# sen-ye/dmvae

Measured on AMD Instinct MI355X. Metric: images/sec DMVAE train step @256x256, higher is better.
Workload: dtype bf16

## Files before the change

### dmvae_amd/_lib.py

```python
from __future__ import annotations

import ctypes
import os
from ctypes import POINTER, Structure, c_char_p, c_float, c_int, c_int32, c_longlong, c_size_t, c_uint, c_ulonglong, c_void_p

_HERE = os.path.dirname(os.path.abspath(__file__))
LIB_PATH = os.environ.get("DMVAE_LIB") or os.path.join(_HERE, "libdmvae_hip.so")


class ConvDesc(Structure):
    _fields_ = [("n", c_int32), ("h", c_int32), ("w", c_int32), ("cin", c_int32), ("cout", c_int32),
                ("ks", c_int32), ("upsample", c_int32), ("act", c_int32), ("out_f32", c_int32), ("stride", c_int32), ("transposed", c_int32),
                ("w_layout", c_int32)]


class PackEntry(Structure):
    _fields_ = [("src", c_void_p), ("dst", c_void_p), ("dst2", c_void_p),
                ("cout", c_int32), ("cin", c_int32), ("T", c_int32), ("rows_pad", c_int32), ("cols_pad", c_int32), ("mode", c_int32), ("subpixel", c_int32),
                ("reserved", c_int32), ("start", c_ulonglong), ("count", c_ulonglong)]


class WtEntry(Structure):
    _fields_ = [("src", c_void_p), ("dst", c_void_p), ("N", c_int32), ("K", c_int32), ("start", c_uint), ("tiles_x", c_uint)]


class OdeTerms(Structure):
    _fields_ = [("k", c_void_p * 7), ("c", c_float * 7), ("nk", c_int32), ("k_bf16", c_int32)]


ABI_VERSION = 9

SIGNATURES = {
    "dmvae_last_error": (c_char_p, []),
    "dmvae_abi_version": (c_int, []),
    "dmvae_rms_modulate_fwd_f32": (c_int, [c_void_p] * 6 + [c_size_t, c_int, c_int, c_int, c_float, c_void_p]),
    "dmvae_rms_modulate_bwd_f32": (c_int, [c_void_p] * 8 + [c_size_t, c_int, c_int, c_int, c_void_p]),
    "dmvae_layernorm_bwd_full_f32": (c_int, [c_void_p] * 5 + [c_size_t, c_int, c_float, c_void_p]),
    "dmvae_bcast_rows_f32": (c_int, [c_int] + [c_void_p] * 4 + [c_size_t, c_int, c_int, c_int, c_void_p]),
    "dmvae_colsum_groups_f32": (c_int, [c_void_p, c_void_p, c_int, c_int, c_int, c_int, c_void_p]),
    "dmvae_swiglu_fwd_f32": (c_int, [c_void_p, c_void_p, c_size_t, c_int, c_void_p]),
    "dmvae_swiglu_bwd_f32": (c_int, [c_void_p, c_void_p, c_void_p, c_size_t, c_int, c_void_p]),
    "dmvae_qknorm_rope_fwd_f32": (c_int, [c_void_p] * 9 + [c_int] * 5 + [c_float, c_void_p]),
    "dmvae_qknorm_rope_bwd_f32": (c_int, [c_void_p] * 12 + [c_int] * 5 + [c_void_p]),
    "dmvae_reparam_kl_workspace": (c_size_t, [c_size_t, c_int]),
    "dmvae_reparam_kl_fwd": (c_int, [c_void_p] * 5 + [c_size_t, c_size_t, c_int, c_int, c_void_p]),
    "dmvae_reparam_kl_bwd": (c_int, [c_void_p] * 4 + [c_float, c_void_p, c_size_t, c_int, c_int, c_void_p]),
    "dmvae_conv2d_nhwc_fwd": (c_int, [c_void_p, c_void_p, c_void_p, c_void_p, c_void_p, POINTER(ConvDesc), c_void_p]),
    "dmvae_conv2d_nhwc_fwd_gnstats_workspace": (c_size_t, [POINTER(ConvDesc), c_int]),
    "dmvae_conv2d_nhwc_fwd_gnstats": (c_int, [c_void_p] * 7 + [c_size_t, c_int, c_float, POINTER(ConvDesc), c_void_p]),
    "dmvae_conv2d_nhwc_wgrad_workspace": (c_size_t, [POINTER(ConvDesc)]),
    "dmvae_gemm_nt_batched": (c_int, [c_void_p] * 5 + [c_int] * 4 + [c_longlong] * 3 + [c_int, c_int, c_void_p]),
    "dmvae_gemm_tn_batched_workspace": (c_size_t, [c_int, c_int, c_int, c_int]),
    "dmvae_gemm_tn_batched": (c_int, [c_void_p] * 4 + [c_size_t] + [c_int] * 4 + [c_longlong] * 3 + [c_float, c_int, c_void_p]),
    "dmvae_set_dynamic": (c_int, [c_int]),
    "dmvae_linear_rows_supported": (c_int, [c_int, c_int, c_int]),
    "dmvae_linear_rows_bf16": (c_int, [c_void_p] * 4 + [c_int] * 10 + [c_void_p]),
    "dmvae_linear_rows_wgrad": (c_int, [c_void_p] * 4 + [c_int] * 6 + [c_void_p]),
    "dmvae_linear_bf16": (c_int, [c_void_p] * 4 + [c_int] * 10 + [c_void_p]),
    "dmvae_linear_bf16_swiglu_pre": (c_int, [c_void_p] * 5 + [c_int] * 9 + [c_void_p]),
    "dmvae_linear_bf16_sk_supported": (c_int, [c_int] * 5),
    "dmvae_linear_bf16_sk_workspace": (c_size_t, [c_int] * 5),
    "dmvae_linear_bf16_sk": (c_int, [c_void_p] * 5 + [c_size_t] + [c_int] * 11 + [c_void_p]),
    "dmvae_linear_bf16_batched_supported": (c_int, [c_int] * 4),
    "dmvae_linear_bf16_batched": (c_int, [c_void_p] * 3 + [c_int] * 7 + [c_longlong] * 3 + [c_int, c_void_p]),
    "dmvae_linear_bf16_plan": (c_int, [c_int, c_int, c_int, POINTER(c_int), POINTER(c_int)]),
    "dmvae_linear_weight_t_kmajor": (c_int, [c_void_p, c_void_p, c_int, c_int, c_void_p]),
    "dmvae_pack_entry_bytes": (c_size_t, []),
    "dmvae_pack_weights_batched": (c_int, [c_void_p, c_int, c_ulonglong, c_int, c_void_p]),
    "dmvae_softmax_rows_fwd": (c_int, [c_void_p, c_void_p, c_int, c_int, c_float, c_void_p]),
    "dmvae_softmax_rows_bwd": (c_int, [c_void_p, c_void_p, c_void_p, c_int, c_int, c_float, c_void_p]),
    "dmvae_transpose_bf16": (c_int, [c_void_p, c_void_p, c_int, c_int, c_int, c_void_p]),
    "dmvae_pack_conv_weight": (c_int, [c_void_p, c_void_p] + [c_int] * 6 + [c_void_p]),
    "dmvae_pack_conv_weight_v2": (c_int, [c_void_p, c_void_p, c_void_p] + [c_int] * 6 + [c_void_p]),
    "dmvae_conv_halo_applies": (c_int, [POINTER(ConvDesc)]),
    "dmvae_conv_kmajor_applies": (c_int, [POINTER(ConvDesc)]),
    "dmvae_subpixel_weight": (c_int, [c_void_p, c_void_p, c_int, c_int, c_void_p]),
    "dmvae_subpixel_weight_fold": (c_int, [c_void_p, c_void_p, c_int, c_int, c_int, c_void_p]),
    "dmvae_colsum_bf16": (c_int, [c_void_p, c_void_p, c_void_p, c_size_t, c_size_t, c_int, c_int, c_void_p]),
    "dmvae_conv_out_wgrad_workspace": (c_size_t, [c_int, c_int, c_int, c_int, c_int]),
    "dmvae_conv_out_wgrad": (c_int, [c_void_p, c_void_p, c_void_p, c_void_p, c_size_t, c_int, c_int, c_int, c_int, c_int, c_int, c_void_p]),
    "dmvae_sumpool2x2_nhwc": (c_int, [c_void_p, c_void_p, c_int, c_int, c_int, c_int, c_void_p]),
    "dmvae_maxpool2x2_nhwc": (c_int, [c_void_p, c_void_p, c_int, c_int, c_int, c_int, c_void_p]),
    "dmvae_maxpool2x2_relu_bwd_nhwc": (c_int, [c_void_p, c_void_p, c_void_p, c_void_p, c_int, c_int, c_int, c_int, c_void_p]),
    "dmvae_relu_bwd": (c_int, [c_void_p, c_void_p, c_void_p, c_size_t, c_void_p]),
    "dmvae_leaky_relu_bwd": (c_int, [c_void_p, c_void_p, c_void_p, c_size_t, c_float, c_void_p]),
    "dmvae_sde_euler_step": (c_int, [c_void_p, c_void_p, c_int, c_void_p, c_void_p, c_void_p, c_size_t] + [c_float] * 6 + [c_void_p]),
    "dmvae_image_to_u8": (c_int, [c_void_p, c_void_p, c_size_t, c_int, c_int, c_int, c_void_p]),
# ... 159 lines not shown
```

### dmvae_amd/csrc/conv_pp.hip

```cpp
#include "common.h"
#include "dmvae_hip.h"
#include <cstdlib>
#include <atomic>
#include <mutex>
#include <type_traits>
#include <unordered_map>


namespace dmvae_conv_pp {

struct Args {
  const bf16* x;
  const bf16* w;
  const float* bias;
  const bf16* res;
  void* y;
  int N, Hi, Wi, Cin, Ho, Wo, Cout;
  int ks, act, M, ctiles, total;
  int so, pd, sd;
  int Ml;
  unsigned wsRow, wsTap, wsChunk;
  float* gnpart;
  unsigned* sched;
  unsigned long long* dbg;
};

__device__ __forceinline__ int hswz(int row) { return (row >> 1) & 2; }

__device__ __forceinline__ void divmod_small(int m, int d, float inv_d, bool, int& q, int& r) {
  q = (int)((float)m * inv_d);
  r = m - q * d;
  if (r < 0) { q--; r += d; }
  if (r >= d) { q++; r -= d; }
}

template <int TM, int TP, int WM, int WP, int NBUF, bool UPS, bool OUT_F32, bool KO, bool GEN = false, bool SUB = false, bool DYN = false, bool STATS = false,
          bool HALO = false>
__global__ __launch_bounds__(512) void conv_pp_kernel(Args a) {
#if __HIP_DEVICE_COMPILE__
  constexpr int BM = TM / WM / 32, BP = TP / WP / 32;
  constexpr int TILE_A = TM * 64, TILE_B = TP * 64, SLOT = TILE_A + TILE_B;
  constexpr int NPA = TM >= 128 ? TM / 128 : 1, NPB = TP / 128;
  static_assert(TM >= 128 || HALO, "the 64-row tile exists in the halo form only");
  constexpr int NP = NPA + NPB;
  constexpr int PF = NBUF - 1;
  static_assert(WM * WP == 8 && BM * BP == 8, "8 waves x 8 accumulators");
  static_assert(!HALO || (!UPS && !GEN && !SUB && KO && NBUF == 4), "HALO: plain 3x3, chunk-outer K order");
  constexpr int NPH = NPB + 1;
  constexpr int HALO_B = (TP + 16) * 64;
  constexpr int GROUP = 2 * TILE_A + HALO_B;
  constexpr int EPI_OFF = HALO ? GROUP : 2 * SLOT;
  constexpr int EPI_BYTES = 8 * 32 * (((BM >= 4 ? BM / 2 : BM) * 32) * 4 + 16);
  constexpr int DUMP_OFF = GROUP + (GROUP > EPI_BYTES ? GROUP : EPI_BYTES);
  constexpr bool DIRECT = HALO && !OUT_F32;
  constexpr int BM16 = BM * 2, BP16 = BP * 2;
  extern __shared__ __attribute__((aligned(16))) char smem[];

  const int tid = threadIdx.x, lane = tid & 63;
  const int wave = __builtin_amdgcn_readfirstlane(tid >> 6);
  const int grp = wave >> 2;
  const int wm = wave / WP, wp = wave % WP;
  static_assert(!SUB || (!UPS && !GEN && KO), "SUB: its own instantiation, chunk-outer K order");
  const int T = SUB ? 4 : a.ks * a.ks;
  const int TW = SUB ? 16 : T;
  const int nchunk = a.Cin >> 5;
  const int nK = T * nchunk;

  const unsigned wbytes = (unsigned)a.Cout * TW * a.Cin * 2u;
  const unsigned xbytes = (unsigned)a.N * a.Hi * a.Wi * a.Cin * 2u;
  const int SR = GEN ? ((UPS || a.ks == 1) ? 0 : (a.sd == 2 ? 1 : a.pd)) : 1;
  const int sds = GEN && a.sd == 2 ? 1 : 0;
  const unsigned shift = GEN ? ((!UPS && a.ks != 1) ? (unsigned)(SR * a.Wi + SR) * a.Cin * 2u : 0u)
                             : ((!UPS && (SUB || a.ks == 3)) ? (unsigned)(a.Wi + 1) * a.Cin * 2u : 0u);
  const __amdgpu_buffer_rsrc_t rA = dmvae_buffer_rsrc(a.w, wbytes);
  const __amdgpu_buffer_rsrc_t rB =
      dmvae_buffer_rsrc(reinterpret_cast<const char*>(a.x) - shift, xbytes + shift);

  const int dvw = SUB ? a.Wi : a.Wo;
  const int hw = SUB ? a.Hi * a.Wi : a.Ho * a.Wo;
  const float inv_hw = 1.0f / (float)hw, inv_wo = 1.0f / (float)dvw;
  const bool small_m = a.M < (1 << 24);
  int m0 = 0, n0 = 0;
  int par = 0;
  unsigned voffA[NPA];
  unsigned ctrB[NPB], maskB[NPB], selB[NPB];
  unsigned rowo[UPS ? NPB : 1][3], colo[UPS ? NPB : 1][3];
  unsigned ctrH[HALO ? NPH : 1], mskH[HALO ? NPH : 1];
// ... 1 lines not shown
  int it = 0, it_tap = 0, it_ch = 0;
  unsigned soffB_tap = 0;
  auto setup = [&](unsigned work) {
    int lane_s = lane;
    if constexpr (DIRECT) asm volatile("" : "+v"(lane_s));
    const unsigned wid = xcd_remap(work, a.total);
    if constexpr (SUB) {
      const unsigned q = wid / a.ctiles;
      n0 = (int)(wid - q * a.ctiles) * TM;
      par = __builtin_amdgcn_readfirstlane((int)(q & 3u));
      m0 = (int)(q >> 2) * TP;
    } else {
      m0 = (int)(wid / a.ctiles) * TP;
      n0 = (int)(wid % a.ctiles) * TM;
    }
    it = it_tap = it_ch = 0;
    it_ky = 0;
#pragma unroll
    for (int p = 0; p < NPA; p++) {
      const int row = (wave * NPA + p) * 16 + (lane_s >> 2);
      int co = n0 + row;
      if constexpr (DIRECT) {
        constexpr int CW_ = TM / WM;
        const int wmr = row / CW_, rr = row % CW_;
        co = n0 + wmr * CW_ + BM16 * (rr & 15) + (rr >> 4);
      }
      const int c = (lane_s & 3) ^ swz64(row);
      voffA[p] = (co < a.Cout && row < TM) ? (unsigned)co * a.wsRow + c * 16u : SENT;
    }
    if constexpr (HALO) {
#pragma unroll
      for (int q = 0; q < NPH; q++) {
        const int i = (q < NPB ? (wave * NPB + q) * 16 : TP) + (lane_s >> 2);
        const int own = min(max(i - 1, 0), TP - 1);
        const int m = m0 + own;
        const int c = (lane_s & 3) ^ hswz(i);
        unsigned mask = 0;
        if (m < a.M && i < TP + 2 && (q < NPB || wave == 0)) {
          int n, r, y, x;
          divmod_small(m, hw, inv_hw, small_m, n, r);
          divmod_small(r, dvw, inv_wo, small_m, y, x);
          mask = (y > 0 ? 1u : 0u) | 2u | (y < a.Ho - 1 ? 4u : 0u);
          if ((i == 0 && x == 0) || (i == TP + 1 && x == a.Wo - 1)) mask = 0;
        }
        ctrH[q] = (unsigned)(m0 + i) * a.Cin * 2u + c * 16u;
        mskH[q] = mask;
      }
    } else {
#pragma unroll
    for (int p = 0; p < NPB; p++) {
    const int row = (wave * NPB + p) * 16 + (lane_s >> 2);
    const int m = m0 + row;
    const int c = (lane_s & 3) ^ swz64(row);
    unsigned mask = 0;
    ctrB[p] = 0;
    if (m < a.M) {
      int n, r, y, x;
      divmod_small(m, hw, inv_hw, small_m, n, r);
      divmod_small(r, dvw, inv_wo, small_m, y, x);
      int by = y, bx = x;
      if constexpr (SUB) {
        by = y - 1 + (par >> 1); bx = x - 1 + (par & 1);
        const unsigned rm = (by >= 0 ? 0x3u : 0u) | (by + 1 < a.Hi ? 0xCu : 0u);
        const unsigned cm = (bx >= 0 ? 0x5u : 0u) | (bx + 1 < a.Wi ? 0xAu : 0u);
        mask = rm & cm;
      } else if (UPS || !GEN) {
        if (a.ks == 3) {
          const unsigned rm = (y > 0 ? 0x007u : 0u) | 0x038u | (y < a.Ho - 1 ? 0x1C0u : 0u);
          const unsigned cm = (x > 0 ? 0x049u : 0u) | 0x092u | (x < a.Wo - 1 ? 0x124u : 0u);
          mask = rm & cm;
        } else {
          mask = 1;
        }
      } else if (a.ks == 1) {
        mask = 1;
      } else {
// ... 69 lines not shown
        const unsigned co = kx == 0 ? colo[UPS ? p : 0][0] : (kx == 1 ? colo[UPS ? p : 0][1] : colo[UPS ? p : 0][2]);
        v = ro + co;
      }
      selB[p] = ((maskB[p] >> it_tap) & 1u) ? v : SENT;
    }
  };
  auto issue = [&](int slot) {
    const bool live = it < nK;
    if (live && (KO || it_ch == 0)) new_tap();
    unsigned soA = (unsigned)it_tap * a.wsTap + (unsigned)it_ch * a.wsChunk;
    if constexpr (SUB)
      soA = (unsigned)((((par >> 1) + (it_tap & 2)) << 2) + (par & 1) + ((it_tap & 1) << 1)) * a.wsTap + (unsigned)it_ch * a.wsChunk;
    unsigned soB = soffB_tap + (unsigned)it_ch * 64u;
    constexpr bool live_b = true;
    if constexpr (GEN) {
      soA = (unsigned)__builtin_amdgcn_readfirstlane((int)soA);
      soB = (unsigned)__builtin_amdgcn_readfirstlane((int)soB);
    }
#pragma unroll
    for (int p = 0; p < NPA; p++)
      __builtin_amdgcn_raw_ptr_buffer_load_lds(rA, LPTR(smem + slot + (wave * NPA + p) * 1024), 16, live ? voffA[p] : SENT, soA, 0, 0);
#pragma unroll
    for (int p = 0; p < NPB; p++)
      __builtin_amdgcn_raw_ptr_buffer_load_lds(rB, LPTR(smem + slot + TILE_A + (wave * NPB + p) * 1024), 16, (live && live_b) ? selB[p] : SENT, soB, 0, 0);
    it++;
    if (KO) {
      if (++it_tap == T) { it_tap = 0; it_ch++; }
    } else {
      if (++it_ch == nchunk) { it_ch = 0; it_tap++; }
    }
  };

  auto issue_h = [&](auto KXc) __attribute__((always_inline)) {
    constexpr int KX = decltype(KXc)::value;
    const bool live = it < nK;
    const unsigned soA = (unsigned)(it_ky * 3 + KX) * a.wsTap + (unsigned)it_ch * a.wsChunk;
    const int isl = it;
    const int da = ((isl >> 1) & 1) * GROUP + (isl & 1) * TILE_A;
#pragma unroll
    for (int p = 0; p < NPA; p++)
      __builtin_amdgcn_raw_ptr_buffer_load_lds(rA, LPTR(smem + ((wave * NPA + p) * 16 < TM ? da + (wave * NPA + p) * 1024 : DUMP_OFF)), 16, live ? voffA[p] : SENT, soA, 0, 0);
    if constexpr (KX == 0) {
      const unsigned soH = (unsigned)(it_ky * a.Wi) * a.Cin * 2u + (unsigned)it_ch * 64u;
      const int dh = ((it_ch + it_ky) & 1) * GROUP + 2 * TILE_A;
#pragma unroll
      for (int q = 0; q < NPH; q++) {
        const unsigned v = (live && ((mskH[HALO ? q : 0] >> it_ky) & 1u)) ? ctrH[HALO ? q : 0] : SENT;
        const int dst = q < NPB ? dh + (wave * NPB + q) * 1024 : (wave == 0 ? dh + TP * 64 : DUMP_OFF);
        __builtin_amdgcn_raw_ptr_buffer_load_lds(rB, LPTR(smem + dst), 16, v, soH, 0, 0);
      }
    }
    it++;
    if constexpr (KX == 2) {
      if (++it_ky == 3) { it_ky = 0; it_ch++; }
    }
  };
  using K0_ = std::integral_constant<int, 0>; using K1_ = std::integral_constant<int, 1>; using K2_ = std::integral_constant<int, 2>;

  auto stamp = [&](unsigned work, int k) {
    if (a.dbg && tid == 0) a.dbg[(size_t)work * 8 + k] = __builtin_amdgcn_s_memtime();
  };
  auto claim = [&]() {
    if (tid == 0) {
      const unsigned x = blockIdx.x & 7u, first = gridDim.x >> 3;
      unsigned flat = 0xFFFFFFFFu;
      for (unsigned k = 0; k < 8u; k++) {
        const unsigned xx = (x + k) & 7u;
        const unsigned cnt = ((unsigned)a.total >> 3) + (xx < ((unsigned)a.total & 7u) ? 1u : 0u);
        const unsigned j = first + atomicAdd(a.sched + xx, 1u);
        if (j < cnt) { flat = j * 8u + xx; break; }
      }
      __hip_atomic_store(a.sched + 16 + blockIdx.x, flat, __ATOMIC_RELEASE, __HIP_MEMORY_SCOPE_WORKGROUP);
    }
  };
  stamp(blockIdx.x, 0);
  setup(blockIdx.x);
  stamp(blockIdx.x, 1);
  if constexpr (HALO) {
    issue_h(K0_{}); issue_h(K1_{}); issue_h(K2_{});
  } else {
#pragma unroll
    for (int u = 0; u < PF; u++) issue(u * SLOT);
  }
  for (unsigned work = blockIdx.x; work < (unsigned)a.total;) {
  const int m0c = m0, n0c = n0;
  const int parc = par;
  if constexpr (DYN) claim();
  int boffk[HALO ? 3 : 1][HALO ? BP16 : 1];
  if constexpr (HALO) {
    int lane_h = lane;
    asm volatile("" : "+v"(lane_h));
#pragma unroll
    for (int j = 0; j < BP16; j++) {
      const int prow = wp * (TP / WP) + j * 16 + (lane_h & 15);
      int q, x;
      divmod_small(m0c + prow, dvw, inv_wo, small_m, q, x);
      const int zoff = (TP + 2) * 64 + ((lane_h >> 4) << 4);
#pragma unroll
      for (int k = 0; k < 3; k++) {
        const int h = prow + k;
        const int off = h * 64 + (((lane_h >> 4) ^ hswz(h)) << 4);
        boffk[HALO ? k : 0][HALO ? j : 0] = (k == 0 && x == 0) || (k == 2 && x == a.Wo - 1) ? zoff : off;
      }
    }
  }
#pragma unroll
  for (int i = 0; i < BM16; i++)
#pragma unroll
    for (int j = 0; j < BP16; j++)
#pragma unroll
      for (int r = 0; r < 4; r++) acc[i][j][r] = 0.f;
  wait_vmcnt<HALO ? 2 * NPA : (PF - 1) * NP>();
  __builtin_amdgcn_s_barrier();
  stamp(work, 2);
  if (grp == 1) __builtin_amdgcn_s_setprio(1);
  if (grp == 1) __builtin_amdgcn_s_barrier();

  bf16x8 af[BM16], bfr[BP16];
  int slot_rd = 0, slot_wr = PF * SLOT;
  unsigned next_dyn = 0;
  if constexpr (HALO) {
    int ka = 0, sh = 2 * TILE_A;
    auto ktile = [&](auto KXc) __attribute__((always_inline)) {
      constexpr int KX = decltype(KXc)::value;
      const char* sa = smem + ((ka >> 1) & 1) * GROUP + (ka & 1) * TILE_A;
      const char* sb = smem + sh;
#pragma unroll
      for (int j = 0; j < BP16; j++) bfr[j] = *reinterpret_cast<const bf16x8*>(sb + boffk[HALO ? KX : 0][HALO ? j : 0]);
#pragma unroll
      for (int i = 0; i < BM16; i++) af[i] = *reinterpret_cast<const bf16x8*>(sa + aoff[i]);
      issue_h(KXc);
      ka++;
      if constexpr (KX == 2) sh = sh == 2 * TILE_A ? GROUP + 2 * TILE_A : 2 * TILE_A;
      wait_vmcnt<KX == 2 ? 2 * NPA : 2 * NPA + NPH>();
      __builtin_amdgcn_s_waitcnt(0xC07F);
      asm volatile("" ::: "memory");
      __builtin_amdgcn_sched_barrier(0);
      __builtin_amdgcn_s_barrier();
      __builtin_amdgcn_sched_barrier(0);
#pragma unroll
      for (int i = 0; i < BM16; i++)
#pragma unroll
        for (int j = 0; j < BP16; j++) {
          if constexpr (DIRECT) asm volatile("v_mfma_f32_16x16x32_bf16 %0, %1, %2, %0" : "+a"(acc[i][j]) : "v"(bfr[j]), "v"(af[i]));
          else asm volatile("v_mfma_f32_16x16x32_bf16 %0, %1, %2, %0" : "+a"(acc[i][j]) : "v"(af[i]), "v"(bfr[j]));
        }
      __builtin_amdgcn_sched_barrier(0);
      __builtin_amdgcn_s_barrier();
      __builtin_amdgcn_sched_barrier(0);
    };
#pragma unroll 1
    for (int t = 0; t < nK; t += 3) { ktile(K0_{}); ktile(K1_{}); ktile(K2_{}); }
  } else {
#pragma unroll 1
  for (int t = 0; t < nK; t++) {
    const char* sb = smem + slot_rd;
#pragma unroll
    for (int j = 0; j < BP16; j++) bfr[j] = *reinterpret_cast<const bf16x8*>(sb + boff[j]);
#pragma unroll
    for (int i = 0; i < BM16; i++) af[i] = *reinterpret_cast<const bf16x8*>(sb + aoff[i]);
    issue(slot_wr);
    slot_rd = slot_rd + SLOT == NBUF * SLOT ? 0 : slot_rd + SLOT;
    slot_wr = slot_wr + SLOT == NBUF * SLOT ? 0 : slot_wr + SLOT;
    wait_vmcnt<(PF - 1) * NP>();
    __builtin_amdgcn_s_waitcnt(0xC07F);
    asm volatile("" ::: "memory");
    __builtin_amdgcn_sched_barrier(0);
    __builtin_amdgcn_s_barrier();
    __builtin_amdgcn_sched_barrier(0);
#pragma unroll
    for (int i = 0; i < BM16; i++)
#pragma unroll
      for (int j = 0; j < BP16; j++)
        asm volatile("v_mfma_f32_16x16x32_bf16 %0, %1, %2, %0" : "+a"(acc[i][j]) : "v"(af[i]), "v"(bfr[j]));
    __builtin_amdgcn_sched_barrier(0);
    __builtin_amdgcn_s_barrier();
    __builtin_amdgcn_sched_barrier(0);
  }
  }
  stamp(work, 3);
  if (grp == 0) __builtin_amdgcn_s_barrier();
  if constexpr (DYN) next_dyn = __hip_atomic_load(a.sched + 16 + blockIdx.x, __ATOMIC_ACQUIRE, __HIP_MEMORY_SCOPE_WORKGROUP);
  wait_vmcnt<0>();
  asm volatile("s_nop 15\n\ts_nop 15" ::: "memory");

// ... 369 lines not shown
  const unsigned long long key = ((unsigned long long)(unsigned)dev << 56) ^ (unsigned long long)reinterpret_cast<uintptr_t>(st);
  auto it = slot.find(key);
  if (it == slot.end()) {
    int& n = used[dev];
    if (n >= SCHED_SLOTS) return nullptr;
    it = slot.emplace(key, n++).first;
  }
  return b->second + (size_t)it->second * SCHED_WORDS;
}

static std::atomic<int> g_dynamic{-1};
static bool dynamic_on() {
  const int v = g_dynamic.load(std::memory_order_relaxed);
  if (v >= 0) return v != 0;
  static const bool env = [] { const char* e = getenv("DMVAE_PP_DYNAMIC"); return e ? atoi(e) != 0 : false; }();
  return env;
}

template <int TM, int TP, int WM, int WP, int NBUF, bool UPS, bool F32, bool KO, bool GEN = false, bool SUB = false, bool DYN = false, bool STATS = false,
          bool HALO = false>
int launch(Args a, hipStream_t st) {
  a.ctiles = (a.Cout + TM - 1) / TM;
  a.total = ((a.M + TP - 1) / TP) * a.ctiles * (SUB ? 4 : 1);
  constexpr int persist = 256;
  const unsigned grid = (persist > 0 && a.total > persist) ? (unsigned)persist : (unsigned)a.total;
  if constexpr (!DYN && !UPS && KO && !F32) {
    if (dynamic_on() && grid == 256u && (unsigned)a.total > grid) {
      a.sched = sched_for(st);
      if (a.sched) return launch<TM, TP, WM, WP, NBUF, UPS, F32, KO, GEN, SUB, true, STATS, HALO>(a, st);
    }
  }
  constexpr int cwh = (TM / WM / 32 >= 4) ? TM / WM / 2 : TM / WM;
  constexpr int ring = NBUF * (TM + TP) * 64, epi = 2 * (TM + TP) * 64 + 8 * 32 * (cwh * 4 + 16);
  constexpr int group = 2 * TM * 64 + (TP + 16) * 64, epi_h = 8 * 32 * (cwh * 4 + 16);
  constexpr int lds = HALO ? group + (group > epi_h ? group : epi_h) + 1024 : (ring > epi ? ring : epi);
  DMVAE_LDS_OPTIN(lds, conv_pp_kernel<TM, TP, WM, WP, NBUF, UPS, F32, KO, GEN, SUB, DYN, STATS, HALO>);
  hipLaunchKernelGGL((conv_pp_kernel<TM, TP, WM, WP, NBUF, UPS, F32, KO, GEN, SUB, DYN, STATS, HALO>), dim3(grid), dim3(512), lds, st, a);
  DMVAE_CHECK_LAUNCH();
  return 0;
}

static constexpr int halo_mode() { return 3; }
static constexpr bool korder_on() { return true; }
static bool halo_for(int ks, int cout, bool plain, bool ups, bool f32) {
  const int h = halo_mode();
  return plain && !ups && !f32 && ks == 3 && h != 0 && korder_on() && (cout > 128 || (h & 2));
}

template <bool UPS, bool F32>
int pick(const Args& a, hipStream_t st, bool gen) {
  if constexpr (!UPS) {
    if (gen) {
      if (a.Cout <= 128) return launch<128, 512, 2, 4, 4, false, F32, true, true>(a, st);
      return launch<256, 256, 2, 4, 4, false, F32, true, true>(a, st);
    }
  }
  if constexpr (UPS) {
    if (a.Cout <= 128) return launch<128, 512, 2, 4, 4, UPS, F32, false>(a, st);
    return launch<256, 256, 2, 4, 4, UPS, F32, false>(a, st);
  } else {
    if constexpr (!F32) {
      if (halo_for(a.ks, a.Cout, !gen, UPS, F32)) {
        if (a.Cout > 128) return a.gnpart ? launch<256, 256, 2, 4, 4, false, false, true, false, false, false, true, true>(a, st)
                                          : launch<256, 256, 2, 4, 4, false, false, true, false, false, false, false, true>(a, st);
        if (a.Cout <= 64 && !a.gnpart)
          return launch<64, 1024, 1, 8, 4, false, false, true, false, false, false, false, true>(a, st);
        return a.gnpart ? launch<128, 512, 2, 4, 4, false, false, true, false, false, false, true, true>(a, st)
                        : launch<128, 512, 2, 4, 4, false, false, true, false, false, false, false, true>(a, st);
      }
      if (a.gnpart) {
        if (a.Cout <= 128) return launch<128, 512, 2, 4, 4, false, false, true, false, false, false, true>(a, st);
        return launch<256, 256, 2, 4, 4, false, false, true, false, false, false, true>(a, st);
      }
    }
    if (a.Cout <= 128) return launch<128, 512, 2, 4, 4, UPS, F32, true>(a, st);
    return launch<256, 256, 2, 4, 4, UPS, F32, true>(a, st);
  }
}

}

static unsigned long long* g_dbg = nullptr;
extern "C" void dmvae_debug_timing(void* buf) { g_dbg = (unsigned long long*)buf; }

__global__ __launch_bounds__(64) void occupy_kernel(unsigned long long ticks) {
  extern __shared__ char occ[];
  occ[threadIdx.x] = 0;
  const unsigned long long t0 = wall_clock64();
  while (wall_clock64() - t0 < ticks) __builtin_amdgcn_s_sleep(32);
}
extern "C" int dmvae_set_dynamic(int on) {
  dmvae_conv_pp::g_dynamic.store(on < 0 ? -1 : (on != 0), std::memory_order_relaxed);
  return dmvae_conv_pp::dynamic_on() ? 1 : 0;
}

extern "C" int dmvae_debug_occupy(int blocks, int lds_bytes, int microseconds, hipStream_t stream) {
  DMVAE_LDS_OPTIN(160 * 1024, occupy_kernel);
  hipLaunchKernelGGL(occupy_kernel, dim3(blocks), dim3(64), lds_bytes, stream, (unsigned long long)microseconds * 100ull);
  DMVAE_CHECK_LAUNCH();
  return 0;
}

int dmvae_conv_geometry(const dmvae_conv_desc* d, int* ho, int* wo, int* so, int* pd, int* sd, int* fl);

extern "C" int dmvae_conv_halo_applies(const dmvae_conv_desc* d) {
  using namespace dmvae_conv_pp;
  if (!d) return 0;
  int ho, wo, so, pd, sd, fl;
  if (dmvae_conv_geometry(d, &ho, &wo, &so, &pd, &sd, &fl) != 0) return 0;
  const bool plain = !(d->upsample == 2 || d->stride == 2 || d->ks == 4 || d->transposed);
  const long long M = (long long)d->n * ho * wo;
  const long long xbytes = (long long)d->n * d->h * d->w * d->cin * 2;
  const long long wbytes = (long long)d->cout * d->ks * d->ks * d->cin * 2;
  constexpr long long min_m = 16384;
  if (d->cin % 32 != 0 || d->cout < 64 || d->cout % 8 != 0 || M < min_m || xbytes + (1ll << 22) >= (1ll << 31) || wbytes >= (1ll << 31)) return 0;
  if (M >= (1ll << 24) || M * d->cout * (d->out_f32 ? 4 : 2) >= (1ll << 31)) return 0;
  return halo_for(d->ks, d->cout, plain, fl != 0, d->out_f32 != 0) ? 1 : 0;
}

extern "C" int dmvae_conv_kmajor_applies(const dmvae_conv_desc* d) {
  using namespace dmvae_conv_pp;
  if (!d) return 0;
  int ho, wo, so, pd, sd, fl;
  if (dmvae_conv_geometry(d, &ho, &wo, &so, &pd, &sd, &fl) != 0) return 0;
  const bool plain = !(d->upsample == 2 || d->stride == 2 || d->ks == 4 || d->transposed);
  const long long M = (long long)d->n * ho * wo;
  const long long xbytes = (long long)d->n * d->h * d->w * d->cin * 2;
  const long long wbytes = (long long)d->cout * d->ks * d->ks * d->cin * 2;
  constexpr long long min_m = 16384;
  if (d->cin % 32 != 0 || d->cout < 64 || d->cout % 8 != 0 || M < min_m || xbytes + (1ll << 22) >= (1ll << 31) || wbytes >= (1ll << 31)) return 0;
  if (M >= (1ll << 24) || M * d->cout * (d->out_f32 ? 4 : 2) >= (1ll << 31)) return 0;
  return 1;
}

int dmvae_conv_pp_try(const void* x, const void* w, const void* bias, const void* residual, void* y, const dmvae_conv_desc* d,
                      hipStream_t stream, float* gnpart, int gn_groups, int* gn_tp) {
  if (gn_tp) *gn_tp = 0;
  using namespace dmvae_conv_pp;
  int ho, wo, so, pd, sd, fl;
  if (dmvae_conv_geometry(d, &ho, &wo, &so, &pd, &sd, &fl) != 0) return 1;
  const bool plain = !(d->upsample == 2 || d->stride == 2 || d->ks == 4 || d->transposed);
  const bool sub = d->transposed && d->ks == 4 && d->stride == 2;
  const int ups = fl ? 1 : 0;
  const long long M = (long long)d->n * ho * wo;
  const long long xbytes = (long long)d->n * d->h * d->w * d->cin * 2;
  const long long wbytes = (long long)d->cout * d->ks * d->ks * d->cin * 2;
  constexpr long long min_m = 16384;
  if (d->cin % 32 != 0 || d->cout < 64 || d->cout % 8 != 0 || M < min_m || xbytes + (1ll << 22) >= (1ll << 31) || wbytes >= (1ll << 31)) return 1;
  if (M >= (1ll << 24)) return 1;
  if (M * d->cout * (d->out_f32 ? 4 : 2) >= (1ll << 31)) return 1;
  if (d->w_layout != 0 && d->w_layout != 1) {
    dmvae_set_error("conv2d_nhwc_fwd: w_layout %d (0 = tap-major, 1 = K-tile-major where dmvae_conv_kmajor_applies(d) is 1)", d->w_layout);
    return -1;
  }
  Args a;
  a.wsRow = d->w_layout ? 64u : (unsigned)(d->ks * d->ks * d->cin) * 2u;
  a.wsTap = d->w_layout ? (unsigned)d->cout * 64u : (unsigned)d->cin * 2u;
  a.wsChunk = d->w_layout ? (unsigned)(d->ks * d->ks) * (unsigned)d->cout * 64u : 64u;
  a.x = (const bf16*)x; a.w = (const bf16*)w; a.bias = (const float*)bias; a.res = (const bf16*)residual; a.y = y;
  a.N = d->n; a.Hi = d->h; a.Wi = d->w; a.Cin = d->cin; a.Cout = d->cout;
  a.Ho = ho; a.Wo = wo; a.so = so; a.pd = pd; a.sd = sd;
  a.ks = d->ks; a.act = d->act; a.M = (int)M; a.ctiles = 0; a.dbg = g_dbg;
  a.Ml = d->n * d->h * d->w;
  a.gnpart = nullptr;
  if (gnpart && gn_tp && !d->out_f32 && (plain || sub) && !ups && gn_groups > 0 && d->cout % gn_groups == 0 && (d->cout / gn_groups) % 4 == 0) {
    const int tp = d->cout <= 128 ? 512 : 256;
    const long long per_image = sub ? (long long)d->h * d->w : (long long)ho * wo;
    if (per_image % tp == 0) { a.gnpart = gnpart; *gn_tp = tp; }
  }
  a.sched = nullptr;
  const bool f32 = d->out_f32 != 0;
  if (sub) {
    a.M = a.Ml;
    if (a.gnpart) {
      if (a.Cout <= 128) return launch<128, 512, 2, 4, 4, false, false, true, false, true, false, true>(a, stream);
      return launch<256, 256, 2, 4, 4, false, false, true, false, true, false, true>(a, stream);
    }
    if (a.Cout <= 128) return f32 ? launch<128, 512, 2, 4, 4, false, true, true, false, true>(a, stream) : launch<128, 512, 2, 4, 4, false, false, true, false, true>(a, stream);
    return f32 ? launch<256, 256, 2, 4, 4, false, true, true, false, true>(a, stream) : launch<256, 256, 2, 4, 4, false, false, true, false, true>(a, stream);
  }
  if (ups) return f32 ? pick<true, true>(a, stream, false) : pick<true, false>(a, stream, false);
  return f32 ? pick<false, true>(a, stream, !plain) : pick<false, false>(a, stream, !plain);
}
```

### dmvae_amd/ops.py

```python
from __future__ import annotations

import ctypes
import os
from typing import Optional, Sequence, Tuple

import torch

from . import _lib, parity
from ._lib import ConvDesc, check

bf16 = torch.bfloat16
f32 = torch.float32

ACT_NONE, ACT_SILU, ACT_RELU, ACT_RELU_GATE, ACT_LEAKY, ACT_GELU = 0, 1, 2, 3, 4, 5
ACT_SWIGLU = 6


def _stream() -> int:
    return torch.cuda.current_stream().cuda_stream


def _req(t: torch.Tensor, dtype, name: str) -> torch.Tensor:
    if not t.is_cuda:
        raise _lib.DmvaeHipError(f"{name}: expected a GPU tensor; dmvae_amd has no CPU path")
    if t.dtype != dtype:
        raise TypeError(f"{name}: expected {dtype}, got {t.dtype}")
    if not t.is_contiguous():
        raise ValueError(f"{name}: tensor must be contiguous")
    return t


def _ptr(t: Optional[torch.Tensor]):
    return None if t is None else t.data_ptr()


_WS = {}

KERNEL_TIMING = None
_PP_HALO = 3


def workspace(nbytes: int, device, slot: str = "main") -> torch.Tensor:
    key = (device.index if device.index is not None else torch.cuda.current_device(), _stream(), slot)
    ws = _WS.get(key)
    if ws is None or ws.numel() < nbytes:
        ws = torch.empty(max(int(nbytes), 1 << 20), dtype=torch.uint8, device=device)
        _WS[key] = ws
    return ws


def pack_conv_weight(w: torch.Tensor, for_dgrad: bool = False, rows_pad: int = 0, cols_pad: int = 0, kmajor: bool = False) -> torch.Tensor:
    if parity.on():
        return parity.pack_conv_weight(w, for_dgrad, rows_pad, cols_pad)
    w = _req(w, f32, "weight")
    if w.dim() == 2:
        cout, cin, ks = w.shape[0], w.shape[1], 1
    else:
        cout, cin, ks = w.shape[0], w.shape[1], w.shape[2]
    rows, cols = (cin, cout) if for_dgrad else (cout, cin)
    rows_pad, cols_pad = max(rows_pad, rows), max(cols_pad, cols)
    out = torch.empty(rows_pad, ks * ks, cols_pad, dtype=bf16, device=w.device)
    out2 = torch.empty(cols_pad // 32, ks * ks, rows_pad, 32, dtype=bf16, device=w.device) if (kmajor and cols_pad % 32 == 0) else None
    check(_lib.lib().dmvae_pack_conv_weight_v2(w.data_ptr(), out.data_ptr(), _ptr(out2), cout, cin, ks, rows_pad, cols_pad, int(for_dgrad), _stream()),
          "pack_conv_weight")
    if out2 is not None:
        out._dmvae_kmajor = out2
    return out


def _weight_operand(w_packed: torch.Tensor, d) -> int:
    wk = getattr(w_packed, "_dmvae_kmajor", None)
    if wk is not None and _lib.lib().dmvae_conv_kmajor_applies(ctypes.byref(d)):
# ... 14 lines not shown
def subpixel_weight_fold(dwd: torch.Tensor, dw_out: Optional[torch.Tensor] = None, accumulate: bool = False) -> torch.Tensor:
    dwd = _req(dwd, f32, "dwd")
    cin, cout = dwd.shape[0], dwd.shape[1]
    dw = dw_out if dw_out is not None else torch.empty(cout, cin, 3, 3, dtype=f32, device=dwd.device)
    assert dw.is_contiguous() and dw.numel() == cout * cin * 9
    check(_lib.lib().dmvae_subpixel_weight_fold(dwd.data_ptr(), dw.data_ptr(), cout, cin, int(accumulate), _stream()), "subpixel_weight_fold")
    return dw


def colsum(x: torch.Tensor, out: Optional[torch.Tensor] = None, accumulate: bool = False) -> torch.Tensor:
    c = x.shape[-1]
    if x.dtype == f32 and parity.on():
        s = parity.colsum(x.reshape(-1, c))
        if out is None:
            return s
        return out.add_(s) if accumulate else out.copy_(s)
    x = _req(x, bf16, "x")
    out = out if out is not None else torch.empty(c, dtype=f32, device=x.device)
    ws = workspace(512 * c * 4, x.device, slot="colsum")
    check(_lib.lib().dmvae_colsum_bf16(x.data_ptr(), out.data_ptr(), ws.data_ptr(), ws.numel(), x.numel() // c, c, int(accumulate), _stream()), "colsum_bf16")
    return out


def conv_out_size(h: int, w: int, ks: int, upsample: int = 0, stride: int = 1, transposed: bool = False):
    if ks == 4:
        return ((h - 1) * stride + 2, (w - 1) * stride + 2) if transposed else ((h - 2) // stride + 1, (w - 2) // stride + 1)
    if upsample or transposed:
        return 2 * h, 2 * w
    return (h // 2, w // 2) if stride == 2 else (h, w)


def _conv_label(n, ho, wo, cin, cout, ks, upsample, out_f32, stride, transposed, stats):
    sub = bool(transposed) and ks == 4 and stride == 2
    if cin % 32 == 0 and cout >= 64 and cout % 8 == 0 and n * ho * wo >= 16384:
        ups1 = int(upsample) == 1
        gen = (int(upsample) == 2 or stride == 2 or ks == 4 or bool(transposed)) and not sub
        t = lambda f: "true" if f else "false"
        dyn = os.environ.get("DMVAE_PP_DYNAMIC", "0") not in ("", "0") and not ups1 and not out_f32 and (n * ho * wo // (512 if cout <= 128 else 256)) * ((cout + 255) // 256 if cout > 128 else 1) > 256
        halo = ks == 3 and not gen and not sub and not ups1 and not out_f32
        label = "conv_pp_kernel<%s, %s, %s, %s, %s, %s, %s, %s, %s>" % (("64, 1024, 1, 8, 4" if (halo and cout <= 64 and not stats) else ("128, 512" if cout <= 128 else "256, 256") + ", 2, 4, 4"), t(ups1), t(out_f32),
                                                                       "false" if ups1 else "true", t(gen), t(sub), t(dyn), t(stats), t(halo))
    else:
        label = "conv_fwd_kernel"
    return label, 2.0 * n * ho * wo * cout * cin * (4 if sub else ks * ks)


def conv2d_nhwc(x: torch.Tensor, w_packed: torch.Tensor, bias: Optional[torch.Tensor] = None,
                residual: Optional[torch.Tensor] = None, ks: int = 3, upsample=False, act: int = ACT_NONE,
                out_f32: bool = False, stride: int = 1, transposed: bool = False, flop_channels: Optional[Tuple[int, int]] = None) -> torch.Tensor:
    if x.dtype == f32 and parity.on():
        y = conv2d_nhwc(parity.split_channels(x, parity.A_SIDE), w_packed, bias, None, ks, upsample, ACT_NONE, True, stride, transposed)
        return parity.epilogue(y, residual, act)
    x = _req(x, bf16, "x")
    w_packed = _req(w_packed, bf16, "w_packed")
    n, h, w_, cin = x.shape
    cout = w_packed.shape[0]
    assert w_packed.shape[1] == ks * ks and w_packed.shape[2] == cin, (w_packed.shape, ks, cin)
    ho, wo = conv_out_size(h, w_, ks, int(upsample), stride, transposed)
    y = torch.empty(n, ho, wo, cout, dtype=f32 if out_f32 else bf16, device=x.device)
    if bias is not None:
        _req(bias, f32, "bias")
    if residual is not None:
        _req(residual, bf16, "residual")
        assert residual.shape == y.shape
    d = ConvDesc(n, h, w_, cin, cout, ks, int(upsample), act, int(out_f32), stride, int(transposed))
    timing = KERNEL_TIMING
    if timing is not None:
        e0 = torch.cuda.Event(enable_timing=True)
        e0.record()
    check(_lib.lib().dmvae_conv2d_nhwc_fwd(x.data_ptr(), _weight_operand(w_packed, d), _ptr(bias), _ptr(residual), y.data_ptr(), ctypes.byref(d),
                                           _stream()), "conv2d_nhwc_fwd")
    if timing is not None:
# ... 1691 lines not shown
```

### include/dmvae_hip.h

```cpp
#ifndef DMVAE_HIP_H
#define DMVAE_HIP_H

#include <stddef.h>
#include <stdint.h>

#ifdef __cplusplus
extern "C" {
#endif

typedef struct ihipStream_t* dmvae_stream_t;

const char* dmvae_last_error(void);
int dmvae_abi_version(void);


typedef struct dmvae_conv_desc {
  int32_t n, h, w;
  int32_t cin, cout;
  int32_t ks;
  int32_t upsample;
  int32_t act;
  int32_t out_f32;
  int32_t stride;
  int32_t transposed;
// ... 52 lines not shown
int dmvae_norm_conv_out_bwd(const void* dy, const void* w, const void* x, const void* stats, const void* gamma, const void* beta, void* dx, void* dgamma,
                            void* dbeta, void* workspace, size_t workspace_bytes, int n, int h, int wd, int c, int groups, int cout, int accumulate,
                            dmvae_stream_t stream);

int dmvae_groupnorm_short_supported(int n, int hw, int c, int cs, int groups);
int dmvae_groupnorm_apply_short(const void* x, const void* stats, const void* gamma, const void* beta, const void* w, const void* bias, void* a, void* xs,
                                int n, int hw, int c, int cs, int groups, int act, dmvae_stream_t stream);
size_t dmvae_groupnorm_bwd_short_workspace(int n, int hw, int c, int cs, int groups);
int dmvae_groupnorm_bwd_short(const void* da, const void* x, const void* dys, const void* wt, const void* stats, const void* gamma, const void* beta,
                              void* dx, void* dgamma, void* dbeta, void* colsum, void* workspace, size_t workspace_bytes, int n, int hw, int c, int cs,
                              int groups, int act, int accumulate, int colsum_accumulate, dmvae_stream_t stream);

int dmvae_conv_in3_supported(int n, int h, int w, int cout);
size_t dmvae_conv_in3_workspace(int n, int h, int w);
int dmvae_conv_in3(const void* x0, const void* x1, int n0, const void* shift, const void* scale, const void* w, const void* bias, void* y,
                   void* workspace, size_t workspace_bytes, int n, int h, int wd, int cout, int act, dmvae_stream_t stream);


int dmvae_gemm_nt_batched(const void* A, const void* B, const void* bias, const void* R, void* C, int M, int N,
                          int K, int batch, long long a_bs, long long b_bs, long long c_bs, int act, int out_f32,
                          dmvae_stream_t stream);

size_t dmvae_gemm_tn_batched_workspace(int M, int N, int K, int batch);
int dmvae_gemm_tn_batched(const void* A, const void* B, void* C, void* workspace, size_t workspace_bytes, int M,
                          int N, int K, int batch, long long a_bs, long long b_bs, long long c_bs, float alpha,
                          int out_f32, dmvae_stream_t stream);

int dmvae_linear_rows_supported(int M, int N, int K);
int dmvae_linear_rows_bf16(const void* x, const void* w, const void* bias, void* y, int M, int N, int K, int ldx, int ldw, int ldy, int act,
                           int bias_bf16, int out_f32, int w_layout, dmvae_stream_t stream);
int dmvae_linear_rows_wgrad(const void* dy, const void* x, void* dw, void* db, int M, int N, int K, int lddy, int ldx, int accumulate, dmvae_stream_t stream);

int dmvae_set_dynamic(int on);

int dmvae_linear_bf16(const void* x, const void* w, const void* bias, void* y, int M, int N, int K, int lda, int ldw, int ldy,
                      int act, int bias_bf16, int out_f32, int w_layout, dmvae_stream_t stream);
int dmvae_linear_bf16_plan(int M, int N, int K, int* tile_cols, int* tile_rows);
int dmvae_linear_bf16_batched_supported(int batch, int M, int N, int K);
int dmvae_linear_bf16_batched(const void* x, const void* w, void* y, int batch, int M, int N, int K, int lda, int ldw, int ldy, long long sx, long long sw,
                              long long sy, int out_f32, dmvae_stream_t stream);
int dmvae_linear_bf16_swiglu_pre(const void* x, const void* w, const void* bias, void* g, void* x12, int M, int N, int K, int lda, int ldw, int ldg,
                                 int ldx12, int bias_bf16, int w_layout, dmvae_stream_t stream);

int dmvae_linear_bf16_sk_supported(int M, int N, int K, int splits, int tile);
size_t dmvae_linear_bf16_sk_workspace(int M, int N, int K, int splits, int tile);
int dmvae_linear_bf16_sk(const void* x, const void* w, const void* bias, void* y, void* workspace, size_t workspace_bytes, int splits, int tile,
                         int M, int N, int K, int lda, int ldw, int ldy, int act, int bias_bf16, int w_layout, dmvae_stream_t stream);
int dmvae_linear_weight_t_kmajor(const void* w, void* out, int N, int K, dmvae_stream_t stream);

int dmvae_softmax_rows_fwd(const void* s, void* p, int rows, int cols, float scale, dmvae_stream_t stream);
int dmvae_softmax_rows_bwd(const void* dp, const void* p, void* ds, int rows, int cols, float scale,
                           dmvae_stream_t stream);
int dmvae_transpose_bf16(const void* src, void* dst, int batch, int rows, int cols, dmvae_stream_t stream);


int dmvae_pack_conv_weight(const void* w, void* out, int cout, int cin, int ks, int rows_pad, int cols_pad,
                           int for_dgrad, dmvae_stream_t stream);
int dmvae_pack_conv_weight_v2(const void* w, void* out, void* out_kmajor, int cout, int cin, int ks, int rows_pad, int cols_pad,
                              int for_dgrad, dmvae_stream_t stream);
typedef struct {
  const float* src; void* dst; void* dst2;
  int32_t cout, cin, T, rows_pad, cols_pad, mode, subpixel, reserved;
  uint64_t start, count;
} dmvae_pack_entry;
size_t dmvae_pack_entry_bytes(void);
int dmvae_pack_weights_batched(const void* table, int n_entries, unsigned long long total, int max_taps, dmvae_stream_t stream);
// ... 250 lines not shown
```

Measured before the change: 493.1.

## Extend halo-strip staging to sub-pixel transposed conv 2x2 per-parity kernel

The halo input-strip scheme, previously limited to plain 3x3 convs, now also covers the sub-pixel (per-parity 2x2) transposed conv at the 256x256 tile. It loads two row strips per channel chunk and reuses them across the horizontal taps, where each tap used to issue its own B-tile load. This cuts global-to-LDS traffic and load instructions for transposed convs with Cout above 128. It adds LDS use for the second strip and new masking and wait-count logic that could be wrong at edges. A runtime mode switch is also added, and it is on by default.

```diff
diff --git a/dmvae_amd/_lib.py b/dmvae_amd/_lib.py
--- a/dmvae_amd/_lib.py
+++ b/dmvae_amd/_lib.py
@@ -53,6 +53,7 @@
     "dmvae_gemm_tn_batched_workspace": (c_size_t, [c_int, c_int, c_int, c_int]),
     "dmvae_gemm_tn_batched": (c_int, [c_void_p] * 4 + [c_size_t] + [c_int] * 4 + [c_longlong] * 3 + [c_float, c_int, c_void_p]),
     "dmvae_set_dynamic": (c_int, [c_int]),
+    "dmvae_conv_pp_halo_mode": (c_int, [c_int]),
     "dmvae_linear_rows_supported": (c_int, [c_int, c_int, c_int]),
     "dmvae_linear_rows_bf16": (c_int, [c_void_p] * 4 + [c_int] * 10 + [c_void_p]),
     "dmvae_linear_rows_wgrad": (c_int, [c_void_p] * 4 + [c_int] * 6 + [c_void_p]),
diff --git a/dmvae_amd/csrc/conv_pp.hip b/dmvae_amd/csrc/conv_pp.hip
--- a/dmvae_amd/csrc/conv_pp.hip
+++ b/dmvae_amd/csrc/conv_pp.hip
@@ -45,14 +45,19 @@
   constexpr int NP = NPA + NPB;
   constexpr int PF = NBUF - 1;
   static_assert(WM * WP == 8 && BM * BP == 8, "8 waves x 8 accumulators");
-  static_assert(!HALO || (!UPS && !GEN && !SUB && KO && NBUF == 4), "HALO: plain 3x3, chunk-outer K order");
+  static_assert(!HALO || (!UPS && !GEN && KO && NBUF == 4), "HALO: plain 3x3 or the per-parity 2x2 form, chunk-outer K order");
+  static_assert(!(HALO && SUB) || (TM == 256 && TP == 256 && !OUT_F32), "SUB + HALO: the 256 x 256 tile with a bf16 result");
+  constexpr int HK = SUB ? 2 : 3;
+  constexpr int HY = SUB ? 2 : 1;
+  constexpr int GT = HK * HY;
   constexpr int NPH = NPB + 1;
-  constexpr int HALO_B = (TP + 16) * 64;
+  constexpr int STRIP_B = (TP + 16) * 64;
+  constexpr int HALO_B = HY * STRIP_B;
   constexpr int GROUP = 2 * TILE_A + HALO_B;
   constexpr int EPI_OFF = HALO ? GROUP : 2 * SLOT;
   constexpr int EPI_BYTES = 8 * 32 * (((BM >= 4 ? BM / 2 : BM) * 32) * 4 + 16);
   constexpr int DUMP_OFF = GROUP + (GROUP > EPI_BYTES ? GROUP : EPI_BYTES);
-  constexpr bool DIRECT = HALO && !OUT_F32;
+  constexpr bool DIRECT = HALO && !OUT_F32 && !SUB;
   constexpr int BM16 = BM * 2, BP16 = BP * 2;
   extern __shared__ __attribute__((aligned(16))) char smem[];
 
@@ -120,16 +125,22 @@
 #pragma unroll
       for (int q = 0; q < NPH; q++) {
         const int i = (q < NPB ? (wave * NPB + q) * 16 : TP) + (lane_s >> 2);
-        const int own = min(max(i - 1, 0), TP - 1);
+        const int own = min(max(SUB ? i - 1 + (par & 1) : i - 1, 0), TP - 1);
         const int m = m0 + own;
         const int c = (lane_s & 3) ^ hswz(i);
         unsigned mask = 0;
-        if (m < a.M && i < TP + 2 && (q < NPB || wave == 0)) {
+        if (m < a.M && i < (SUB ? TP + 1 : TP + 2) && (q < NPB || wave == 0)) {
           int n, r, y, x;
           divmod_small(m, hw, inv_hw, small_m, n, r);
           divmod_small(r, dvw, inv_wo, small_m, y, x);
+          if constexpr (SUB) {
+            const int by = y - 1 + (par >> 1);
+            mask = (by >= 0 ? 1u : 0u) | (by + 1 < a.Hi ? 2u : 0u);
+            if (((par & 1) == 0 && i == 0 && x == 0) || ((par & 1) == 1 && i == TP && x == a.Wi - 1)) mask = 0;
+          } else {
           mask = (y > 0 ? 1u : 0u) | 2u | (y < a.Ho - 1 ? 4u : 0u);
           if ((i == 0 && x == 0) || (i == TP + 1 && x == a.Wo - 1)) mask = 0;
+          }
         }
         ctrH[q] = (unsigned)(m0 + i) * a.Cin * 2u + c * 16u;
         mskH[q] = mask;
@@ -265,15 +276,30 @@
   };
 
   auto issue_h = [&](auto KXc) __attribute__((always_inline)) {
-    constexpr int KX = decltype(KXc)::value;
+    constexpr int U = decltype(KXc)::value;
+    constexpr int KX = SUB ? (U & 1) : U, KYS = SUB ? (U >> 1) : 0;
     const bool live = it < nK;
-    const unsigned soA = (unsigned)(it_ky * 3 + KX) * a.wsTap + (unsigned)it_ch * a.wsChunk;
+    unsigned soA = (unsigned)(it_ky * 3 + KX) * a.wsTap + (unsigned)it_ch * a.wsChunk;
+    if constexpr (SUB)
+      soA = (unsigned)((((par >> 1) + 2 * KYS) << 2) + (par & 1) + 2 * KX) * a.wsTap + (unsigned)it_ch * a.wsChunk;
     const int isl = it;
     const int da = ((isl >> 1) & 1) * GROUP + (isl & 1) * TILE_A;
 #pragma unroll
     for (int p = 0; p < NPA; p++)
       __builtin_amdgcn_raw_ptr_buffer_load_lds(rA, LPTR(smem + ((wave * NPA + p) * 16 < TM ? da + (wave * NPA + p) * 1024 : DUMP_OFF)), 16, live ? voffA[p] : SENT, soA, 0, 0);
-    if constexpr (KX == 0) {
+    if constexpr (U == 0 && SUB) {
+#pragma unroll
+      for (int s = 0; s < HY; s++) {
+        const unsigned soH = (unsigned)(((par >> 1) + s) * a.Wi + (par & 1)) * a.Cin * 2u + (unsigned)it_ch * 64u;
+        const int dh = (it_ch & 1) * GROUP + 2 * TILE_A + s * STRIP_B;
+#pragma unroll
+        for (int q = 0; q < NPH; q++) {
+          const unsigned v = (live && ((mskH[HALO ? q : 0] >> s) & 1u)) ? ctrH[HALO ? q : 0] : SENT;
+          const int dst = q < NPB ? dh + (wave * NPB + q) * 1024 : (wave == 0 ? dh + TP * 64 : DUMP_OFF);
+          __builtin_amdgcn_raw_ptr_buffer_load_lds(rB, LPTR(smem + dst), 16, v, soH, 0, 0);
+        }
+      }
+    } else if constexpr (KX == 0 && !SUB) {
       const unsigned soH = (unsigned)(it_ky * a.Wi) * a.Cin * 2u + (unsigned)it_ch * 64u;
       const int dh = ((it_ch + it_ky) & 1) * GROUP + 2 * TILE_A;
 #pragma unroll
@@ -284,11 +310,12 @@
       }
     }
     it++;
-    if constexpr (KX == 2) {
-      if (++it_ky == 3) { it_ky = 0; it_ch++; }
+    if constexpr (U == GT - 1) {
+      if constexpr (SUB) it_ch++;
+      else if (++it_ky == 3) { it_ky = 0; it_ch++; }
     }
   };
-  using K0_ = std::integral_constant<int, 0>; using K1_ = std::integral_constant<int, 1>; using K2_ = std::integral_constant<int, 2>;
+  using K0_ = std::integral_constant<int, 0>; using K1_ = std::integral_constant<int, 1>; using K2_ = std::integral_constant<int, 2>; using K3_ = std::integral_constant<int, 3>;
 
   auto stamp = [&](unsigned work, int k) {
     if (a.dbg && tid == 0) a.dbg[(size_t)work * 8 + k] = __builtin_amdgcn_s_memtime();
@@ -319,7 +346,7 @@
   const int m0c = m0, n0c = n0;
   const int parc = par;
   if constexpr (DYN) claim();
-  int boffk[HALO ? 3 : 1][HALO ? BP16 : 1];
+  int boffk[HALO ? HK : 1][HALO ? BP16 : 1];
   if constexpr (HALO) {
     int lane_h = lane;
     asm volatile("" : "+v"(lane_h));
@@ -330,9 +357,12 @@
       divmod_small(m0c + prow, dvw, inv_wo, small_m, q, x);
       const int zoff = (TP + 2) * 64 + ((lane_h >> 4) << 4);
 #pragma unroll
-      for (int k = 0; k < 3; k++) {
+      for (int k = 0; k < HK; k++) {
         const int h = prow + k;
         const int off = h * 64 + (((lane_h >> 4) ^ hswz(h)) << 4);
+        if constexpr (SUB)
+          boffk[HALO ? k : 0][HALO ? j : 0] = (k == 0 && (parc & 1) == 0 && x == 0) || (k == 1 && (parc & 1) == 1 && x == a.Wi - 1) ? zoff : off;
+        else
         boffk[HALO ? k : 0][HALO ? j : 0] = (k == 0 && x == 0) || (k == 2 && x == a.Wo - 1) ? zoff : off;
       }
     }
@@ -355,17 +385,18 @@
   if constexpr (HALO) {
     int ka = 0, sh = 2 * TILE_A;
     auto ktile = [&](auto KXc) __attribute__((always_inline)) {
-      constexpr int KX = decltype(KXc)::value;
+      constexpr int U = decltype(KXc)::value;
+      constexpr int KX = SUB ? (U & 1) : U;
       const char* sa = smem + ((ka >> 1) & 1) * GROUP + (ka & 1) * TILE_A;
-      const char* sb = smem + sh;
+      const char* sb = smem + sh + (SUB ? (U >> 1) * STRIP_B : 0);
 #pragma unroll
       for (int j = 0; j < BP16; j++) bfr[j] = *reinterpret_cast<const bf16x8*>(sb + boffk[HALO ? KX : 0][HALO ? j : 0]);
 #pragma unroll
       for (int i = 0; i < BM16; i++) af[i] = *reinterpret_cast<const bf16x8*>(sa + aoff[i]);
-      issue_h(KXc);
+      issue_h(std::integral_constant<int, (U + 3) % GT>{});
       ka++;
-      if constexpr (KX == 2) sh = sh == 2 * TILE_A ? GROUP + 2 * TILE_A : 2 * TILE_A;
-      wait_vmcnt<KX == 2 ? 2 * NPA : 2 * NPA + NPH>();
+      if constexpr (U == GT - 1) sh = sh == 2 * TILE_A ? GROUP + 2 * TILE_A : 2 * TILE_A;
+      wait_vmcnt<2 * NPA + (((U + 2) % GT == 0 ? 1 : 0) + ((U + 3) % GT == 0 ? 1 : 0)) * HY * NPH>();
       __builtin_amdgcn_s_waitcnt(0xC07F);
       asm volatile("" ::: "memory");
       __builtin_amdgcn_sched_barrier(0);
@@ -383,7 +414,10 @@
       __builtin_amdgcn_sched_barrier(0);
     };
 #pragma unroll 1
-    for (int t = 0; t < nK; t += 3) { ktile(K0_{}); ktile(K1_{}); ktile(K2_{}); }
+    for (int t = 0; t < nK; t += GT) {
+      ktile(K0_{}); ktile(K1_{}); ktile(K2_{});
+      if constexpr (GT == 4) ktile(K3_{});
+    }
   } else {
 #pragma unroll 1
   for (int t = 0; t < nK; t++) {
@@ -819,7 +853,7 @@
   }
   constexpr int cwh = (TM / WM / 32 >= 4) ? TM / WM / 2 : TM / WM;
   constexpr int ring = NBUF * (TM + TP) * 64, epi = 2 * (TM + TP) * 64 + 8 * 32 * (cwh * 4 + 16);
-  constexpr int group = 2 * TM * 64 + (TP + 16) * 64, epi_h = 8 * 32 * (cwh * 4 + 16);
+  constexpr int group = 2 * TM * 64 + (SUB ? 2 : 1) * (TP + 16) * 64, epi_h = 8 * 32 * (cwh * 4 + 16);
   constexpr int lds = HALO ? group + (group > epi_h ? group : epi_h) + 1024 : (ring > epi ? ring : epi);
   DMVAE_LDS_OPTIN(lds, conv_pp_kernel<TM, TP, WM, WP, NBUF, UPS, F32, KO, GEN, SUB, DYN, STATS, HALO>);
   hipLaunchKernelGGL((conv_pp_kernel<TM, TP, WM, WP, NBUF, UPS, F32, KO, GEN, SUB, DYN, STATS, HALO>), dim3(grid), dim3(512), lds, st, a);
@@ -828,6 +862,9 @@
 }
 
 static constexpr int halo_mode() { return 3; }
+static std::atomic<int> g_halo_sel{4};
+static bool sub_halo_on() { return (g_halo_sel.load(std::memory_order_relaxed) & 4) != 0; }
+static long long min_pixels() { return (g_halo_sel.load(std::memory_order_relaxed) & 8) ? 1 : 16384; }
 static constexpr bool korder_on() { return true; }
 static bool halo_for(int ks, int cout, bool plain, bool ups, bool f32) {
   const int h = halo_mode();
@@ -881,6 +918,11 @@
   return dmvae_conv_pp::dynamic_on() ? 1 : 0;
 }
 
+extern "C" int dmvae_conv_pp_halo_mode(int mode) {
+  if (mode >= 0) dmvae_conv_pp::g_halo_sel.store(mode & 12, std::memory_order_relaxed);
+  return dmvae_conv_pp::halo_mode() | dmvae_conv_pp::g_halo_sel.load(std::memory_order_relaxed);
+}
+
 extern "C" int dmvae_debug_occupy(int blocks, int lds_bytes, int microseconds, hipStream_t stream) {
   DMVAE_LDS_OPTIN(160 * 1024, occupy_kernel);
   hipLaunchKernelGGL(occupy_kernel, dim3(blocks), dim3(64), lds_bytes, stream, (unsigned long long)microseconds * 100ull);
@@ -899,7 +941,7 @@
   const long long M = (long long)d->n * ho * wo;
   const long long xbytes = (long long)d->n * d->h * d->w * d->cin * 2;
   const long long wbytes = (long long)d->cout * d->ks * d->ks * d->cin * 2;
-  constexpr long long min_m = 16384;
+  const long long min_m = min_pixels();
   if (d->cin % 32 != 0 || d->cout < 64 || d->cout % 8 != 0 || M < min_m || xbytes + (1ll << 22) >= (1ll << 31) || wbytes >= (1ll << 31)) return 0;
   if (M >= (1ll << 24) || M * d->cout * (d->out_f32 ? 4 : 2) >= (1ll << 31)) return 0;
   return halo_for(d->ks, d->cout, plain, fl != 0, d->out_f32 != 0) ? 1 : 0;
@@ -914,7 +956,7 @@
   const long long M = (long long)d->n * ho * wo;
   const long long xbytes = (long long)d->n * d->h * d->w * d->cin * 2;
   const long long wbytes = (long long)d->cout * d->ks * d->ks * d->cin * 2;
-  constexpr long long min_m = 16384;
+  const long long min_m = min_pixels();
   if (d->cin % 32 != 0 || d->cout < 64 || d->cout % 8 != 0 || M < min_m || xbytes + (1ll << 22) >= (1ll << 31) || wbytes >= (1ll << 31)) return 0;
   if (M >= (1ll << 24) || M * d->cout * (d->out_f32 ? 4 : 2) >= (1ll << 31)) return 0;
   return 1;
@@ -932,7 +974,7 @@
   const long long M = (long long)d->n * ho * wo;
   const long long xbytes = (long long)d->n * d->h * d->w * d->cin * 2;
   const long long wbytes = (long long)d->cout * d->ks * d->ks * d->cin * 2;
-  constexpr long long min_m = 16384;
+  const long long min_m = min_pixels();
   if (d->cin % 32 != 0 || d->cout < 64 || d->cout % 8 != 0 || M < min_m || xbytes + (1ll << 22) >= (1ll << 31) || wbytes >= (1ll << 31)) return 1;
   if (M >= (1ll << 24)) return 1;
   if (M * d->cout * (d->out_f32 ? 4 : 2) >= (1ll << 31)) return 1;
@@ -959,10 +1001,13 @@
   const bool f32 = d->out_f32 != 0;
   if (sub) {
     a.M = a.Ml;
+    const bool strips = sub_halo_on() && !f32 && a.Cout > 128;
     if (a.gnpart) {
       if (a.Cout <= 128) return launch<128, 512, 2, 4, 4, false, false, true, false, true, false, true>(a, stream);
+      if (strips) return launch<256, 256, 2, 4, 4, false, false, true, false, true, false, true, true>(a, stream);
       return launch<256, 256, 2, 4, 4, false, false, true, false, true, false, true>(a, stream);
     }
+    if (strips) return launch<256, 256, 2, 4, 4, false, false, true, false, true, false, false, true>(a, stream);
     if (a.Cout <= 128) return f32 ? launch<128, 512, 2, 4, 4, false, true, true, false, true>(a, stream) : launch<128, 512, 2, 4, 4, false, false, true, false, true>(a, stream);
     return f32 ? launch<256, 256, 2, 4, 4, false, true, true, false, true>(a, stream) : launch<256, 256, 2, 4, 4, false, false, true, false, true>(a, stream);
   }
diff --git a/dmvae_amd/ops.py b/dmvae_amd/ops.py
--- a/dmvae_amd/ops.py
+++ b/dmvae_amd/ops.py
@@ -37,7 +37,13 @@
 _WS = {}
 
 KERNEL_TIMING = None
-_PP_HALO = 3
+_PP_HALO = 7
+
+
+def conv_pp_halo_mode(mode: int = -1) -> int:
+    global _PP_HALO
+    _PP_HALO = int(_lib.lib().dmvae_conv_pp_halo_mode(int(mode)))
+    return _PP_HALO
 
 
 def workspace(nbytes: int, device, slot: str = "main") -> torch.Tensor:
@@ -118,12 +124,12 @@
 
 def _conv_label(n, ho, wo, cin, cout, ks, upsample, out_f32, stride, transposed, stats):
     sub = bool(transposed) and ks == 4 and stride == 2
-    if cin % 32 == 0 and cout >= 64 and cout % 8 == 0 and n * ho * wo >= 16384:
+    if cin % 32 == 0 and cout >= 64 and cout % 8 == 0 and n * ho * wo >= (1 if _PP_HALO & 8 else 16384):
         ups1 = int(upsample) == 1
         gen = (int(upsample) == 2 or stride == 2 or ks == 4 or bool(transposed)) and not sub
         t = lambda f: "true" if f else "false"
         dyn = os.environ.get("DMVAE_PP_DYNAMIC", "0") not in ("", "0") and not ups1 and not out_f32 and (n * ho * wo // (512 if cout <= 128 else 256)) * ((cout + 255) // 256 if cout > 128 else 1) > 256
-        halo = ks == 3 and not gen and not sub and not ups1 and not out_f32
+        halo = (ks == 3 and not gen and not sub and not ups1 and not out_f32) or (sub and bool(_PP_HALO & 4) and cout > 128 and not out_f32)
         label = "conv_pp_kernel<%s, %s, %s, %s, %s, %s, %s, %s, %s>" % (("64, 1024, 1, 8, 4" if (halo and cout <= 64 and not stats) else ("128, 512" if cout <= 128 else "256, 256") + ", 2, 4, 4"), t(ups1), t(out_f32),
                                                                        "false" if ups1 else "true", t(gen), t(sub), t(dyn), t(stats), t(halo))
     else:
diff --git a/include/dmvae_hip.h b/include/dmvae_hip.h
--- a/include/dmvae_hip.h
+++ b/include/dmvae_hip.h
@@ -108,6 +108,8 @@
 int dmvae_linear_rows_wgrad(const void* dy, const void* x, void* dw, void* db, int M, int N, int K, int lddy, int ldx, int accumulate, dmvae_stream_t stream);
 
 int dmvae_set_dynamic(int on);
+
+int dmvae_conv_pp_halo_mode(int mode);
 
 int dmvae_linear_bf16(const void* x, const void* w, const void* bias, void* y, int M, int N, int K, int lda, int ldw, int ldy,
                       int act, int bias_bf16, int out_f32, int w_layout, dmvae_stream_t stream);
```

Result: no change. 493.9 (median of 6 runs) (+0.2%).
